# JessicaLeu-code/MotionPlanning_5D_m

Measured on AMD Instinct MI355X. Metric: CFS iterations/sec, 5-DoF 30-wp 8-obs batch-1024; l_inf wp err vs quadprog, higher is better.
Workload: dtype f64

## Files before the change

### motionplanning_5d_m_amd/csrc/cfs_device.h

```cpp
#pragma once
#include <hip/hip_runtime.h>
#include <stdint.h>
#include "../../include/cfs_hip.h"

#define CFS_WAVE 64

struct DevRobot {
    int kind;
    int nlink;
    double dh_d[CFS_MAX_LINKS];
    double dh_a[CFS_MAX_LINKS];
    double ca[CFS_MAX_LINKS];
    double sa[CFS_MAX_LINKS];
    double th_off[CFS_MAX_LINKS];
    double base[3];
    double cap[CFS_MAX_LINKS * 6];
    double t2l[CFS_MAX_LINKS * 3];
    double shift_bound;
    double prune_tol;
};
static_assert(sizeof(DevRobot) % 8 == 0, "DevRobot is copied to LDS as doubles");

struct DevCost {
    double Qp[36], Qv[36], Rs[36];
    double qc, ws, wt, pad;
};
static_assert(sizeof(DevCost) % 8 == 0, "DevCost is read as doubles");

struct DistArmParams {
    const DevRobot *rb;
    int N, nobs, nj;
    const double *theta;
    const double *obs;
    double *d;
    int *linkid;
    double *pos;
    double *grad;
};
void launch_dist_arm(const DistArmParams &p, hipStream_t s);
void launch_dist_arm_grad(const DistArmParams &p, hipStream_t s);

struct OrderParams {
    const DevRobot *rb;
    int B, H, nj, nobs;
    int obs_stride;
    int wp_stride;
    const double *x_init;
    const double *obs;
    const double *margin;
    int *key;
    int *order;
};
void launch_order(const OrderParams &p, hipStream_t s);

struct DenseConParams {
    int B, H, nj, nobs;
    double dt;
    const double *dist, *grad;
    const double *u;
    const double *xR1;
    const double *lim, *margin;
    double *Ainq;
    double *binq;
    const double *plim;
};
void launch_dense_con(const DenseConParams &p, hipStream_t s);

struct ClearParams {
    const DevRobot *rb;
    int B, H, nj, nobs, S;
    int move;
    double dt;
    const double *x_, *u, *xR1, *obs;
    double *dist_wp, *dist_path, *dist_lower, *t_path;
    int *link_path;
    int obs_stride, out_stride;
    double rho[CFS_MAX_LINKS * CFS_MAX_LINKS];
};
hipError_t launch_clearance(const ClearParams &p, hipStream_t s);
void cfs_clear_build_rho(const DevRobot &rb, int nj, double *rho);

enum { QP_OK = 0, QP_INFEASIBLE = 2, QP_NUMERIC = 3 };

struct GemvParams {
    int B, nn;
    const double *M;
    const double *X;
    double *Y;
    double scale;
};
void launch_batched_gemv(const GemvParams &p, hipStream_t s);

struct FusedParams {
    const DevRobot *rb;
    int B, H, nobs, mode, has_bounds, max_o_iter, noise_rows;
    int qy, lin_w;
    unsigned rc_nseg, rc_tile, rc_last;
    double dt, alpha, epsilon_O;
    double lmax_vel;
    double polish_tol;
    double lmax_H;
    const double *M1, *M2, *M3;
    const double *QQ;
    const DevCost *cost;
    const double *lim, *maxin, *margin;
    const double *x_init, *xR1, *ff, *caug, *obs, *noise;
    const double *x0;
    double *u, *x_, *cost_all, *e_cost_all, *e_u_all;
    int *iter_O, *total_iter, *status;
    double *Yg;
    double *Pt;
    size_t pt_stride;
    int *pool_flag;
    int pool_n;
    double *dbg;
    int dbg_b, dbg_cap;
    const int *order;
    unsigned long long *stamps;
    int opt;
    double *u_hist;
    double *u_log;
    int nmesh;
    const double *ext_dist;
    const double *ext_grad;
    int resume;
    int max_launch_iters;
    double *st_qu;
    double *st_cost;
    int *st_noise, *st_done;
    int warm_max;
    int piece;
    int no_prune;
    double *dump_dist;
    double *dump_grad;
    int *dump_linkid;
    double *dump_lambda;
};
struct SoftParams {
    double inv_weight;
    double *viol;
    int *n_soft;
};
enum FusedTier { FUSED_W1, FUSED_W2M, FUSED_W2S };
template <FusedTier T, bool JAC, bool SOFT, bool MOVE, bool LIM>
hipError_t launch_fused_tier(int nj, FusedParams p, hipStream_t s, const SoftParams *sp);
template <FusedTier T> bool fused_fits_tier(int nj, int H, int nobs, bool move = false, bool lim = false);
hipError_t launch_fused(int nj, FusedParams p, hipStream_t s, bool force_w1 = false, bool analytic = false, const SoftParams *soft = nullptr,
                        bool move = false, bool lim = false);
bool fused_fits(int nj, int H, int nobs);
bool fused_fits_move(int nj, int H, int nobs, int mode, bool lim = false);
bool fused_fits_lim(int nj, int H, int nobs, int mode, bool move);

struct CostHistParams {
    int B, nn, max_o_iter;
    const double *u_hist, *qu_hist;
    const double *ff, *caug;
    const int *iter_O;
    double *cost_all, *e_cost_all;
};
void launch_cost_history(const CostHistParams &p, hipStream_t s);

struct TermsParams {
    int B, H, nj;
    const double *F1, *F2;
    const double *Cq;
    const double *x0, *xg;
    const double *route;
    int nwp;
    const int *nwp_b;
    int nwp_stride;
    double dt;
    double *x_init, *xR1, *ff, *caug;
};
void launch_build_terms(const TermsParams &p, hipStream_t s);
```

### motionplanning_5d_m_amd/csrc/cfs_fused.hip

```cpp
#include "cfs_geom_dev.h"
#include <algorithm>
#include <atomic>
#include <type_traits>

namespace {

#define STAMP_IF(k) if (P.stamps) { const unsigned long long t_ = clock64(); if (tid == 0) s_acc[k] += t_ - t0_; t0_ = t_; }
#define STAMP(k) do { STAMP_IF(k) } while (0)

constexpr int CERT_AT = 6;
#ifndef CFS_WG_PER_CU
#define CFS_WG_PER_CU 1
#endif
#ifndef CFS_MOVE
#define CFS_MOVE 0
#endif
#ifndef CFS_LIM
#define CFS_LIM 0
#endif
constexpr double REF_A = 1e-4;
constexpr double REF_B = 1e-9;
constexpr int MV_BATCH = 16;
#ifndef CFS_TU
#define CFS_TU 8
#endif
#ifndef CFS_PR
#define CFS_PR 64
#endif
#ifndef CFS_P_LDS
#define CFS_P_LDS 0
#endif
#if CFS_P_LDS
constexpr int P_LDS_MAX_QB = 160;
#endif
static_assert(CFS_PR % 8 == 0 && CFS_PR >= 8, "register-resident P columns come in chunks of 8");
constexpr int FT = 256;
constexpr double DEP_TOL_F = 1e-8;
enum { CT_COL = 0, CT_VELP = 1, CT_VELM = 2, CT_BNDP = 3, CT_BNDM = 4, CT_POSP = 5, CT_POSM = 6 };
__device__ __forceinline__ int mk_code(int type, int i, int jc) { return (type << 16) | (i << 8) | jc; }
__host__ __device__ constexpr unsigned rcp31(unsigned d) { return (unsigned)(0x80000000ull / d) + 1u; }
__device__ __forceinline__ int rcp_div(int e, unsigned rc) { return (int)__umulhi((unsigned)e << 1, rc); }
#define CFS_RCP_DECODE (CFS_WG_PER_CU > 1)

template <int CTRL, int RM>
__device__ __forceinline__ double dpp_f64(double old, double src)
{
    const int rl = __builtin_amdgcn_update_dpp(__double2loint(old), __double2loint(src), CTRL, RM, 0xf, false);
    const int rh = __builtin_amdgcn_update_dpp(__double2hiint(old), __double2hiint(src), CTRL, RM, 0xf, false);
    return __hiloint2double(rh, rl);
}
__device__ __forceinline__ double readlane_f64(double v, int lane)
{
    return __hiloint2double(__builtin_amdgcn_readlane(__double2hiint(v), lane), __builtin_amdgcn_readlane(__double2loint(v), lane));
}
__device__ __forceinline__ double wave_min(double v)
{
    v = fmin(v, dpp_f64<0x111, 0xf>(v, v));
    v = fmin(v, dpp_f64<0x112, 0xf>(v, v));
    v = fmin(v, dpp_f64<0x114, 0xf>(v, v));
    v = fmin(v, dpp_f64<0x118, 0xf>(v, v));
    v = fmin(v, dpp_f64<0x142, 0xa>(v, v));
    v = fmin(v, dpp_f64<0x143, 0xc>(v, v));
    return readlane_f64(v, 63);
}
__device__ __forceinline__ double wave_add(double v)
{
    v += dpp_f64<0x111, 0xf>(0.0, v);
    v += dpp_f64<0x112, 0xf>(0.0, v);
    v += dpp_f64<0x114, 0xf>(0.0, v);
    v += dpp_f64<0x118, 0xf>(0.0, v);
    v += dpp_f64<0x142, 0xa>(0.0, v);
    v += dpp_f64<0x143, 0xc>(0.0, v);
    return readlane_f64(v, 63);
}

__device__ __forceinline__ void sync_rows(bool one_wave)
{
    if (one_wave) {
        __builtin_amdgcn_fence(__ATOMIC_RELEASE, "wavefront");
        __builtin_amdgcn_wave_barrier();
        __builtin_amdgcn_fence(__ATOMIC_ACQUIRE, "wavefront");
    } else __syncthreads();
}

__device__ __forceinline__ void block_argmin(double &v, int &id, double *red, int tid)
{
    const double m = wave_min(v);
    const unsigned long long hit = __ballot(v == m);
    const int src = hit ? (int)__builtin_ctzll(hit) : 0;
    const int mid = __builtin_amdgcn_readlane(id, src);
    const int wv = tid >> 6;
    if ((tid & 63) == 0) { red[wv] = m; reinterpret_cast<int *>(red + FT / 64)[wv] = mid; }
    __syncthreads();
    double bm = red[0];
    int bi = reinterpret_cast<int *>(red + FT / 64)[0];
#pragma unroll
    for (int w = 1; w < FT / 64; ++w) {
        const double om = red[w];
        const int oi = reinterpret_cast<int *>(red + FT / 64)[w];
        if (om < bm) { bm = om; bi = oi; }
    }
    v = bm; id = bi;
}
__device__ __forceinline__ double block_sum(double v, double *red, int tid)
{
    const double s = wave_add(v);
    if ((tid & 63) == 0) red[tid >> 6] = s;
    __syncthreads();
    double t = red[0];
#pragma unroll
    for (int w = 1; w < FT / 64; ++w) t += red[w];
    return t;
}

__device__ __forceinline__ void block_sum4(double &a, double &b, double &c, double &d, double *red, int tid)
{
    const double sa = wave_add(a), sb = wave_add(b), sc = wave_add(c), sd = wave_add(d);
    if ((tid & 63) == 0) { const int w = tid >> 6; red[w] = sa; red[4 + w] = sb; red[8 + w] = sc; red[12 + w] = sd; }
    __syncthreads();
    a = (red[0] + red[1]) + (red[2] + red[3]);
    b = (red[4] + red[5]) + (red[6] + red[7]);
    c = (red[8] + red[9]) + (red[10] + red[11]);
    d = (red[12] + red[13]) + (red[14] + red[15]);
}

__device__ __forceinline__ void block_sum3(double &a, double &b, double &c, double *red, int tid)
{
    const double sa = wave_add(a), sb = wave_add(b), sc = wave_add(c);
    if ((tid & 63) == 0) { const int w = tid >> 6; red[w] = sa; red[4 + w] = sb; red[8 + w] = sc; }
    __syncthreads();
    a = (red[0] + red[1]) + (red[2] + red[3]);
    b = (red[4] + red[5]) + (red[6] + red[7]);
    double t = red[8];
#pragma unroll
    for (int w = 1; w < FT / 64; ++w) t += red[8 + w];
    c = t;
}

__device__ __forceinline__ double wave_scan_incl(double v)
{
    v += dpp_f64<0x111, 0xf>(0.0, v);
    v += dpp_f64<0x112, 0xf>(0.0, v);
    v += dpp_f64<0x114, 0xf>(0.0, v);
    v += dpp_f64<0x118, 0xf>(0.0, v);
    v += dpp_f64<0x142, 0xa>(0.0, v);
    v += dpp_f64<0x143, 0xc>(0.0, v);
    return v;
}

__device__ __forceinline__ double half_scan_incl(double v)
{
    v += dpp_f64<0x111, 0xf>(0.0, v);
    v += dpp_f64<0x112, 0xf>(0.0, v);
    v += dpp_f64<0x114, 0xf>(0.0, v);
    v += dpp_f64<0x118, 0xf>(0.0, v);
    v += dpp_f64<0x142, 0xa>(0.0, v);
    return v;
}

template <int NJ>
__device__ __forceinline__ void roll_lds(double *buf, int H, double dt, int tid)
{
    const int HN = H * NJ;
    if (H <= 32) {
        const int lane = tid & 31;
        for (int c = tid >> 5; c < NJ; c += 2 * (FT / 64)) {
            const double x = lane < H ? buf[lane * NJ + c] : 0.0;
            const double sv = dt * half_scan_incl(x);
            const double sp = dt * half_scan_incl(sv) - (0.5 * dt) * sv;
            if (lane < H) { buf[HN + lane * NJ + c] = sv; buf[2 * HN + lane * NJ + c] = sp; }
        }
        return;
    }
    const int lane = tid & 63, wv = tid >> 6;
    for (int c = wv; c < NJ; c += FT / 64) {
        const double x = lane < H ? buf[lane * NJ + c] : 0.0;
        const double sv = dt * wave_scan_incl(x);
        const double sp = dt * wave_scan_incl(sv) - (0.5 * dt) * sv;
        if (lane < H) { buf[HN + lane * NJ + c] = sv; buf[2 * HN + lane * NJ + c] = sp; }
    }
}

template <int NJ, bool LIM = false>
__device__ __forceinline__ double ndot(int code, const double *buf, const double *g, int H)
{
    const int type = code >> 16, i = (code >> 8) & 0xff, jc = code & 0xff, HN = H * NJ;
    if constexpr (LIM) {
        if (type == CT_POSP) return -buf[2 * HN + i * NJ + jc];
        if (type == CT_POSM) return buf[2 * HN + i * NJ + jc];
    }
    switch (type) {
    case CT_COL: {
        double s = 0.0;
#pragma unroll
        for (int c = 0; c < NJ; ++c) s += g[(jc * H + i) * NJ + c] * buf[2 * HN + i * NJ + c];
        return s;
    }
    case CT_VELP: return -buf[HN + i * NJ + jc];
    case CT_VELM: return buf[HN + i * NJ + jc];
    case CT_BNDP: return -buf[i * NJ + jc];
    default: return buf[i * NJ + jc];
    }
}

template <int NJ, bool LIM = false>
__device__ __forceinline__ double slack_of(int code, const double *xs, const double *g, const double *rhs,
                                           const double *lim, const double *v0, const double *maxin, int H, double *bnd,
                                           double dt = 0.0, const double *plim = nullptr)
{
    const int type = code >> 16, i = (code >> 8) & 0xff, jc = code & 0xff, HN = H * NJ;
    if constexpr (LIM) {
        if (type == CT_POSP || type == CT_POSM) {
            const double pos = v0[NJ + jc] + ((double)(i + 1) * dt) * v0[jc];
            if (type == CT_POSP) { const double bb = plim[NJ + jc] - pos; *bnd = bb; return bb - xs[2 * HN + i * NJ + jc]; }
            const double bb = pos - plim[jc]; *bnd = bb; return bb + xs[2 * HN + i * NJ + jc];
        }
    }
    switch (type) {
    case CT_COL: {
        const double rh = rhs[jc * H + i];
        double s = rh;
#pragma unroll
        for (int c = 0; c < NJ; ++c) s += g[(jc * H + i) * NJ + c] * xs[2 * HN + i * NJ + c];
        *bnd = rh;
        return s;
    }
    case CT_VELP: { const double bb = lim[jc] - v0[jc]; *bnd = bb; return bb - xs[HN + i * NJ + jc]; }
    case CT_VELM: { const double bb = lim[jc] + v0[jc]; *bnd = bb; return bb + xs[HN + i * NJ + jc]; }
    case CT_BNDP: { const double bb = maxin[i * NJ + jc]; *bnd = bb; return bb - xs[i * NJ + jc]; }
    default: { const double bb = maxin[i * NJ + jc]; *bnd = bb; return bb + xs[i * NJ + jc]; }
    }
}


__device__ __forceinline__ double ramp_sum(int a, int m)
{
    const int M = m + 1;
    return 0.5 * (double)(M * (2 * a + 1) - m * M);
}
__device__ __forceinline__ double ramp_dot(int a, int b, int m)
{
    const int M = m + 1;
    return 0.25 * (double)(M * (2 * a + 1) * (2 * b + 1) - 2 * (a + b + 1) * m * M + 2 * (m * M * (2 * m + 1) / 3));
}
template <int NJ, bool LIM = false>
__device__ __forceinline__ double gram_ident(int ca, int cp, const double *g, int H, double dt)
{
    const int ta = ca >> 16, ia = (ca >> 8) & 0xff, ja = ca & 0xff;
    const int tp = cp >> 16, ip = (cp >> 8) & 0xff, jp = cp & 0xff;
    const int m = min(ia, ip);
    if constexpr (LIM) {
        const bool pa = ta >= CT_POSP, pp = tp >= CT_POSP;
        if (pa || pp) {
            const double sa = (ta == CT_POSP || ta == CT_VELP) ? -1.0 : 1.0, sp = (tp == CT_POSP || tp == CT_VELP) ? -1.0 : 1.0;
            if (ta == CT_COL) return (sp * g[(ja * H + ia) * NJ + jp]) * ((dt * dt) * (dt * dt) * ramp_dot(ia, ip, m));
            if (tp == CT_COL) return (sa * g[(jp * H + ip) * NJ + ja]) * ((dt * dt) * (dt * dt) * ramp_dot(ia, ip, m));
            if (ja != jp) return 0.0;
            if (pa && pp) return (sa * sp) * ((dt * dt) * (dt * dt) * ramp_dot(ia, ip, m));
            return (sa * sp) * ((dt * dt * dt) * ramp_sum(pa ? ia : ip, m));
        }
    }
    if (ta == CT_COL && tp == CT_COL) {
        double dot = 0.0;
#pragma unroll
        for (int c = 0; c < NJ; ++c) dot += g[(ja * H + ia) * NJ + c] * g[(jp * H + ip) * NJ + c];
        return dot * ((dt * dt) * (dt * dt) * ramp_dot(ia, ip, m));
    }
    if (ta == CT_COL) return g[(ja * H + ia) * NJ + jp] * ((tp == CT_VELP ? -1.0 : 1.0) * (dt * dt * dt) * ramp_sum(ia, m));
    if (tp == CT_COL) return g[(jp * H + ip) * NJ + ja] * ((ta == CT_VELP ? -1.0 : 1.0) * (dt * dt * dt) * ramp_sum(ip, m));
    if (ja != jp) return 0.0;
    return ((ta == tp) ? 1.0 : -1.0) * (dt * dt) * (double)(m + 1);
}

#if CFS_P_LDS
template <int PR, int QB, bool IN_LDS = false>
#else
template <int PR, int QB>
#endif
struct PRow {
    static constexpr int TU = CFS_TU;
    double v[PR];
    __device__ __forceinline__ void zero(double *ptail, int a, int q)
    {
#pragma unroll
        for (int b = 0; b < PR; ++b) v[b] = 0.0;
        for (int b = PR; b < q; ++b) ptail[(b - PR) * QB + a] = 0.0;
    }
    __device__ __forceinline__ double dot(const double *vec, const double *ptail, int a, int q) const
    {
        double s = 0.0;
#pragma unroll
        for (int b0 = 0; b0 < PR; b0 += 8)
            if (b0 < q) {
#pragma unroll
                for (int jj = 0; jj < 8; ++jj) s += v[b0 + jj] * vec[b0 + jj];
                __builtin_amdgcn_sched_barrier(0);
            }
        int b = PR;
        for (; b + TU <= q; b += TU) {
            double t[TU];
#pragma unroll
            for (int jj = 0; jj < TU; ++jj) t[jj] = ptail[(b + jj - PR) * QB + a];
#pragma unroll
            for (int jj = 0; jj < TU; ++jj) s += t[jj] * vec[b + jj];
        }
        for (; b < q; ++b) s += ptail[(b - PR) * QB + a] * vec[b];
        return s;
    }
    __device__ __forceinline__ void axpy(double alpha, const double *vec, double *ptail, int a, int q)
    {
#pragma unroll
        for (int b0 = 0; b0 < PR; b0 += 8)
            if (b0 < q) {
#pragma unroll
                for (int jj = 0; jj < 8; ++jj) v[b0 + jj] += alpha * vec[b0 + jj];
                __builtin_amdgcn_sched_barrier(0);
            }
        int b = PR;
        for (; b + TU <= q; b += TU) {
// ... 225 lines not shown
    return L;
}

template <int NJ, int QB, bool IDENT, bool JAC, bool MOVE, bool LIM, class... Soft>
__global__ __launch_bounds__(FT, CFS_WG_PER_CU) void cfs_solve_fused_kernel(FusedParams P, Soft... soft_params)
{
    constexpr bool SOFT = sizeof...(Soft) > 0;
    static_assert(!SOFT || (sizeof...(Soft) == 1 && (std::is_same_v<Soft, SoftParams> && ...)), "Soft is empty or SoftParams");
    const SoftParams S{soft_params...};
    constexpr int NS = 2 * NJ, NVT = nvt(NJ), NE = 2 * NJ + 1;
    extern __shared__ __attribute__((aligned(16))) double lds[];
    const int b = P.order ? P.order[blockIdx.x] : (int)blockIdx.x, tid = threadIdx.x;
    const int H = P.H, nobs = P.nobs, HN = H * NJ, nn = HN, NX = H * NS;
    const double dt = P.dt;
    constexpr int PR = QB < CFS_PR ? QB : CFS_PR;
    const FusedLayout L = fused_layout(NJ, H, nobs, QB, PR, LIM);
    DevRobot *rb = reinterpret_cast<DevRobot *>(lds + L.rb);
    double *s_ob = lds + L.ob, *s_x = lds + L.x, *s_u = lds + L.u, *s_qu = lds + L.qu, *s_g = lds + L.g;
    double *s_rhs = lds + L.rhs, *xs = lds + L.xs, *s_up = lds + L.up, *wb = lds + L.wb, *zb = lds + L.zb;
    double *s_d = lds + L.d, *s_r = lds + L.r, *s_rho = lds + L.rho, *s_lam = lds + L.lam, *s_prow = lds + L.prow;
    int *s_act = reinterpret_cast<int *>(lds + L.act);
    int *s_free = reinterpret_cast<int *>(lds + L.fre);
    int *s_prev = reinterpret_cast<int *>(lds + L.prev);
    unsigned char *s_flag = reinterpret_cast<unsigned char *>(lds + L.flag);
    unsigned short *s_slot = reinterpret_cast<unsigned short *>(lds + L.slot);
    int *s_code = reinterpret_cast<int *>(lds + L.code);
    double *red_base = lds + L.red;
    int red_sel = 0;
#define red (red_base + 24 * (red_sel ^= 1))
    double *s_lim = lds + L.small, *s_v0 = s_lim + NJ, *s_th0 = s_v0 + NJ, *s_margin = s_th0 + 2 * NJ;
    double *s_plim = s_margin + nobs;
    double *s_mx = lds + L.mx;
    double *s_racc = lds + L.racc;
    int pool_slot;
    {
        int *pubp = reinterpret_cast<int *>(red_base + 63);
        if (tid == 0) {
            int sidx = (int)(((blockIdx.x * 0x9E3779B1u) >> 8) % (unsigned)P.pool_n);
            int probes = 0;
            while (atomicCAS(&P.pool_flag[sidx * 16], 0, 1) != 0) {
                sidx = sidx + 1 == P.pool_n ? 0 : sidx + 1;
                __builtin_amdgcn_s_sleep(2);
                if (++probes > (1 << 22)) { sidx = -1; break; }
            }
            pubp[0] = sidx;
        }
        __syncthreads();
        pool_slot = pubp[0];
        if (pool_slot < 0) {
            if (tid == 0 && P.piece == 0) { P.status[b] = CFS_NUMERIC; P.iter_O[b] = 1; P.total_iter[b] = 0; }
            return;
        }
    }
    double *const s_pt = P.Pt + (size_t)pool_slot * P.pt_stride;
    double *s_Y = lds + L.y;
    const int QY = P.qy;
    double *const Yg = P.Yg + (size_t)pool_slot * nn * nn;
    auto drop_pool = [&]() {
        __syncthreads();
        if (tid == 0) { __threadfence(); atomicExch(&P.pool_flag[pool_slot * 16], 0); }
    };
    int ncon = nobs * H + (P.has_bounds ? 4 : 2) * HN;
    if constexpr (LIM) ncon = nobs * H + 6 * HN;
    const int maxit = 8 * nn + 200;
    if constexpr (LIM) {
        for (int e = tid; e < nobs * H; e += FT) { const int j = e / H; s_code[e] = mk_code(CT_COL, e - j * H, j); }
    } else
    for (int e = tid; e < ncon; e += FT) {
        int code;
        if (e < nobs * H) { const int j = e / H; code = mk_code(CT_COL, e - j * H, j); }
        else {
            const int f2 = e - nobs * H, ty = f2 / HN, k = f2 - ty * HN, i = k / NJ;
            code = mk_code(1 + ty, i, k - i * NJ);
        }
        s_code[e] = code;
    }

    {
        const double *src = reinterpret_cast<const double *>(P.rb);
        for (int e = tid; e < (int)(sizeof(DevRobot) / 8); e += FT) lds[L.rb + e] = src[e];
        if constexpr (!MOVE)
            for (int e = tid; e < nobs * 6; e += FT) s_ob[e] = P.obs[(size_t)b * nobs * 6 + e];
        for (int e = tid; e < NX; e += FT) s_x[e] = P.x_init[(size_t)b * NX + e];
        for (int e = tid; e < HN; e += FT) { s_u[e] = 0.0; s_qu[e] = 0.0; s_mx[e] = P.has_bounds ? P.maxin[e] : 0.0; }
        if (tid < NJ) {
            s_lim[tid] = P.lim[tid];
            s_v0[tid] = P.xR1[(size_t)b * NS + NJ + tid];
            s_th0[tid] = P.xR1[(size_t)b * NS + tid];
        }
        if (tid < nobs) s_margin[tid] = P.margin[tid];
        if constexpr (LIM)
            if (tid < 2 * NJ) s_plim[tid] = P.lim[NJ + tid];
        if (P.cost) {
            const double *csrc = reinterpret_cast<const double *>(P.cost);
            for (int e = tid; e < (int)(sizeof(DevCost) / 8); e += FT) lds[L.cost + e] = csrc[e];
        }
    }
    __syncthreads();
    if (P.has_bounds)
        for (int e = tid; e < HN; e += FT) {
            const int i = e / NJ, c = e - i * NJ;
            double acc = 0.0;
            for (int k = 0; k <= i; ++k) acc += ((double)(i - k) + 0.5) * s_mx[k * NJ + c];
            s_racc[e] = (dt * dt) * acc;
        }
    unsigned long long *s_acc = reinterpret_cast<unsigned long long *>(red_base + 48);
    if (tid < 12) s_acc[tid] = 0ull;
    unsigned long long t0_ = P.stamps ? clock64() : 0ull;
    double cost_new = P.caug[b], cost_old = 100000.0;
    int iter_O = 1, total_iter = 0, noise_row = 0, status = CFS_OK_MAXITER;
    bool done = false;
    const double iw = S.inv_weight;
    int n_soft = 0;
    bool last_soft = false;
    const int nseg = nobs - P.nmesh;
    int launched = 0;
    if (P.resume) {
        for (int e = tid; e < NX; e += FT) s_x[e] = P.x_[(size_t)b * NX + e];
        for (int e = tid; e < HN; e += FT) { s_u[e] = P.u[(size_t)b * nn + e]; s_qu[e] = P.st_qu[(size_t)b * nn + e]; }
        cost_new = P.st_cost[2 * b]; cost_old = P.st_cost[2 * b + 1];
        iter_O = P.iter_O[b]; total_iter = P.total_iter[b]; status = P.status[b];
        noise_row = P.st_noise[b]; done = P.st_done[b] != 0;
        __syncthreads();
    } else if (P.piece == 0) {
        double d2 = 0.0;
        for (int e = tid; e < NX; e += FT) { const double v = s_x[e] - 1.0; d2 += v * v; }
        d2 = block_sum(d2, red, tid);
        if (sqrt(d2) < P.epsilon_O) { done = true; status = CFS_OK_CONVERGED; }
        else if (iter_O > P.max_o_iter) { done = true; status = CFS_OK_MAXITER; }
    } else if (P.piece == 2) {
        for (int e = tid; e < HN; e += FT) s_u[e] = P.u[(size_t)b * nn + e];
        __syncthreads();
    }

#if CFS_P_LDS
    PRow<PR, QB, QB <= P_LDS_MAX_QB> Pr;
#else
    PRow<PR, QB> Pr;
#endif
#if CFS_P_LDS
    static_assert(IDENT, "the P block takes the place of the Y rows: identity Hessian only");
    if constexpr (QB <= P_LDS_MAX_QB) Pr.pl = lds + L.pl;
#endif
    int prev_q = 0;

    while (!done) {
        bool skip = false;
        if (P.piece == 0 && P.mode == CFS_MODE_PSGCFS) {
            skip = fabs(cost_new - cost_old) < 1e-4;
            if (!skip) cost_old = cost_new;
        } else if (P.piece == 0) cost_old = cost_new;
        const int noise_row_now = noise_row;
        if (P.piece == 0 && P.mode == CFS_MODE_PSGCFS && !skip) ++noise_row;
        auto prep = [&](int ph) {
            if (P.piece == 1) return;
            if (ph == 0) { for (int k = tid; k < HN; k += FT) xs[k] = s_u[k]; }
            else if (ph == 1) roll_lds<NJ>(xs, H, dt, tid);
            else if (ph == 2) {
                const bool psg = P.piece == 0 && P.mode == CFS_MODE_PSGCFS;
                const double sc = (double)iter_O * (double)iter_O + 1.0;
                const bool have = P.noise != nullptr && noise_row_now < P.noise_rows;
                for (int k = tid; k < HN; k += FT) {
                    s_up[k] = xs[2 * HN + k];
                    double v;
                    if (psg && skip) v = s_u[k];
                    else if (psg) {
                        const double nz = have ? P.noise[((size_t)b * P.noise_rows + noise_row_now) * nn + k] : 0.0;
                        v = s_u[k] - P.alpha * ((s_qu[k] + P.ff[(size_t)b * nn + k]) + 10.0 * nz / sc);
                    } else v = P.x0[(size_t)b * nn + k];
                    xs[k] = v;
                }
            } else roll_lds<NJ>(xs, H, dt, tid);
        };
        bool prepped = false;
        if constexpr (JAC) {
            if (nseg > 0) {
                const int W = P.lin_w;
                double *s_sc = lds + L.lin;
                double *s_en = s_sc + W * NJ * 6;
                double *s_tw = s_en + W * NJ * 6;
                double *s_bd = s_en + W * NVT * 6;
#define S_OBW (s_bd + W * NJ * nseg)
                for (int w0 = 0; w0 < H; w0 += W) {
                    const int Wc = min(W, H - w0);
#if CFS_RCP_DECODE
                    unsigned rc_n = P.rc_nseg, rc_t = Wc == W ? P.rc_tile : P.rc_last;
                    asm volatile("" : "+s"(rc_n), "+s"(rc_t));
#endif
                    if (w0 == 0) prep(0);
                    if constexpr (MOVE)
                        for (int e = tid; e < Wc * nseg * 6; e += FT) S_OBW[e] = P.obs[((size_t)b * H + w0) * nobs * 6 + e];
                    for (int e = tid; e < Wc * NJ; e += FT) {
                        const int m = e % NJ, wi = e / NJ;
                        double x = s_x[(w0 + wi) * NS + m];
                        x = x - rb->th_off[m];
                        double sn, cs;
                        sincos(x, &sn, &cs);
                        s_sc[e * 2] = sn;
                        s_sc[e * 2 + 1] = cs;
                    }
                    __syncthreads();
                    for (int wi = tid; wi < Wc; wi += FT) arm_chain(rb, NJ, s_sc + wi * NJ * 2, s_en + wi * NJ * 6, s_tw + wi * NJ * 6);
                    if (w0 == 0) prep(1);
                    __syncthreads();
                    STAMP(10);
                    for (int e = tid; e < NJ * Wc * nseg; e += FT) {
#if CFS_RCP_DECODE
                        const int q = rcp_div(e, rc_n), j = e - q * nseg, k0 = rcp_div(e, rc_t), wi = q - k0 * Wc;
#else
                        const int j = e % nseg, wi = (e / nseg) % Wc, k0 = e / (nseg * Wc);
#endif
                        if constexpr (MOVE) s_bd[(wi * NJ + k0) * nseg + j] = seg_seg_dist(s_en + (wi * NJ + k0) * 6, S_OBW + (wi * nseg + j) * 6);
                        else s_bd[(wi * NJ + k0) * nseg + j] = seg_seg_dist(s_en + (wi * NJ + k0) * 6, s_ob + j * 6);
                    }
                    if (w0 == 0) prep(2);
                    __syncthreads();
                    STAMP(0);
                    for (int e = tid; e < Wc * nseg; e += FT) {
#if CFS_RCP_DECODE
                        const int wi = rcp_div(e, rc_n), j = e - wi * nseg;
#else
                        const int j = e % nseg, wi = e / nseg;
#endif
                        double m0 = INFINITY;
                        int lk = 0;
#pragma unroll
                        for (int k1 = 1; k1 <= NJ; ++k1) { const double bk = s_bd[(wi * NJ + k1 - 1) * nseg + j]; if (bk < m0) { m0 = bk; lk = k1; } }
                        if (P.dump_linkid && launched == 0) P.dump_linkid[((size_t)b * nobs + j) * H + w0 + wi] = lk;
                        s_rhs[j * H + w0 + wi] = m0;
                        double *g = s_g + (j * H + w0 + wi) * NJ;
                        if constexpr (MOVE) {
                            if (lk > 0) winner_grad(s_en + (wi * NJ + lk - 1) * 6, s_tw + wi * NJ * 6, lk - 1, NJ, S_OBW + (wi * nseg + j) * 6, g);
                            else for (int m = 0; m < NJ; ++m) g[m] = 0.0;
                        } else {
                            if (lk > 0) winner_grad(s_en + (wi * NJ + lk - 1) * 6, s_tw + wi * NJ * 6, lk - 1, NJ, s_ob + j * 6, g);
                            else for (int m = 0; m < NJ; ++m) g[m] = 0.0;
                        }
                    }
                    if (w0 == 0) { prep(3); prepped = true; }
                    if constexpr (MOVE) __syncthreads();
                    else if (w0 + W >= H) __syncthreads();
                    STAMP(11);
                }
#undef S_OBW
            }
        } else {
            if (nseg > 0) {
                const int W = P.lin_w;
                double *s_sc = lds + L.lin;
                double *s_en = s_sc + W * NJ * 6;
                double *s_bd = s_en + W * NVT * 6;
                double *s_dv = s_bd + W * NJ * nseg;
                unsigned short *s_list = reinterpret_cast<unsigned short *>(s_dv + W * nseg * NE);
#define S_OBW (s_dv + W * nseg * NE + (NJ * W * nseg + 3) / 4)
                int *s_cnt = s_free;
                for (int w0 = 0; w0 < H; w0 += W) {
                    const int Wc = min(W, H - w0);
#if CFS_RCP_DECODE
                    unsigned rc_n = P.rc_nseg, rc_t = Wc == W ? P.rc_tile : P.rc_last;
                    asm volatile("" : "+s"(rc_n), "+s"(rc_t));
#endif
                    if (w0 == 0) prep(0);
                    if constexpr (MOVE)
                        for (int e = tid; e < Wc * nseg * 6; e += FT) S_OBW[e] = P.obs[((size_t)b * H + w0) * nobs * 6 + e];
                    for (int e = tid; e < Wc * NJ * 3; e += FT) {
                        const int var = e % 3, m = (e / 3) % NJ, wi = e / (3 * NJ);
                        double x = s_x[(w0 + wi) * NS + m];
                        if (var == 1) x = x + FD_EPS / 2;
                        else if (var == 2) x = x - FD_EPS / 2;
                        x = x - rb->th_off[m];
                        double sn, cs;
                        sincos(x, &sn, &cs);
                        s_sc[((wi * NJ + m) * 3 + var) * 2] = sn;
                        s_sc[((wi * NJ + m) * 3 + var) * 2 + 1] = cs;
                    }
                    __syncthreads();
                    for (int e = tid; e < Wc * NE; e += FT) {
                        const int ev = e % NE, wi = e / NE;
                        double M[12], Mn[12], e6[6];
#pragma unroll
                        for (int k1 = 1; k1 <= NJ; ++k1) {
                            const int avar = (ev == 2 * k1 - 1) ? 1 : (ev >= 2 * k1 ? 2 : 0);
                            const double sn = s_sc[((wi * NJ + k1 - 1) * 3 + avar) * 2], cs = s_sc[((wi * NJ + k1 - 1) * 3 + avar) * 2 + 1];
                            fk_step(rb, k1 - 1, sn, cs, k1 == 1 ? nullptr : M, Mn);
#pragma unroll
                            for (int qq = 0; qq < 12; ++qq) M[qq] = Mn[qq];
                            if (ev <= 2 * k1) {
                                link_ends(rb, k1 - 1, M, e6);
                                double *dstE = s_en + (wi * NVT + kvoff(k1) + ev) * 6;
#pragma unroll
                                for (int qq = 0; qq < 6; ++qq) dstE[qq] = e6[qq];
                            }
                        }
                    }
                    if (w0 == 0) prep(1);
                    __syncthreads();
                    STAMP(10);
                    for (int e = tid; e < NJ * Wc * nseg; e += FT) {
#if CFS_RCP_DECODE
                        const int q = rcp_div(e, rc_n), j = e - q * nseg, k0 = rcp_div(e, rc_t), wi = q - k0 * Wc;
#else
                        const int j = e % nseg, wi = (e / nseg) % Wc, k0 = e / (nseg * Wc);
#endif
                        if constexpr (MOVE) s_bd[(wi * NJ + k0) * nseg + j] = seg_seg_dist(s_en + (wi * NVT + kvoff(k0 + 1)) * 6, S_OBW + (wi * nseg + j) * 6);
                        else s_bd[(wi * NJ + k0) * nseg + j] = seg_seg_dist(s_en + (wi * NVT + kvoff(k0 + 1)) * 6, s_ob + j * 6);
                    }
                    if (tid < NJ) s_cnt[tid] = 0;
                    if (w0 == 0) prep(2);
                    __syncthreads();
                    for (int e = tid; e < Wc * nseg; e += FT) {
#if CFS_RCP_DECODE
                        const int wi = rcp_div(e, rc_n), j = e - wi * nseg;
#else
                        const int j = e % nseg, wi = e / nseg;
#endif
                        double bk[NJ], m0 = INFINITY;
                        int lk = 0;
#pragma unroll
                        for (int k1 = 1; k1 <= NJ; ++k1) { bk[k1 - 1] = s_bd[(wi * NJ + k1 - 1) * nseg + j]; if (bk[k1 - 1] < m0) { m0 = bk[k1 - 1]; lk = k1; } }
                        if (P.dump_linkid && launched == 0) P.dump_linkid[((size_t)b * nobs + j) * H + w0 + wi] = lk;
                        const double thr = P.no_prune ? INFINITY : fmax(m0, 0.0001) + rb->prune_tol;
#pragma unroll
                        for (int k1 = 1; k1 <= NJ; ++k1)
                            if (bk[k1 - 1] < thr) s_list[(k1 - 1) * W * nseg + atomicAdd(&s_cnt[k1 - 1], 1)] = (unsigned short)((wi << 8) | j);
                        s_dv[e * NE] = m0;
#pragma unroll
                        for (int ev = 1; ev < NE; ++ev) s_dv[e * NE + ev] = INFINITY;
                    }
                    if (w0 == 0) { prep(3); prepped = true; }
                    __syncthreads();
                    STAMP(0);
                    {
                        int offs[NJ + 1];
                        offs[0] = 0;
#pragma unroll
                        for (int k1 = 1; k1 <= NJ; ++k1) offs[k1] = offs[k1 - 1] + s_cnt[k1 - 1] * 2 * k1;
                        for (int e = tid; e < offs[NJ]; e += FT) {
#if CFS_RCP_DECODE
                            int k1 = 1, lo = 0;
                            unsigned rc = 0x80000001u;
#pragma unroll
                            for (int kk = 2; kk <= NJ; ++kk)
                                if (e >= offs[kk - 1]) { k1 = kk; lo = offs[kk - 1]; rc = (unsigned)(0x100000000ull / (2 * kk)) + 1u; }
                            const int r_ = e - lo, ent = (int)__umulhi((unsigned)r_, rc), v = r_ - ent * (2 * k1) + 1;
#else
                            int k1 = 1, ent = 0, v = 1;
#pragma unroll
                            for (int kk = 1; kk <= NJ; ++kk)
                                if (e >= offs[kk - 1] && e < offs[kk]) {
                                    const int r_ = e - offs[kk - 1];
                                    k1 = kk; ent = r_ / (2 * kk); v = r_ - ent * (2 * kk) + 1;
                                }
#endif
                            const int item = s_list[(k1 - 1) * W * nseg + ent], wi = item >> 8, j = item & 255;
                            double dis;
                            if constexpr (MOVE) dis = seg_seg_dist(s_en + (wi * NVT + kvoff(k1) + v) * 6, S_OBW + (wi * nseg + j) * 6);
                            else dis = seg_seg_dist(s_en + (wi * NVT + kvoff(k1) + v) * 6, s_ob + j * 6);
                            double *dv = s_dv + (wi * nseg + j) * NE;
                            const int evhi = (v == 2 * k1) ? NE - 1 : v;
                            for (int ev = v; ev <= evhi; ++ev)
                                __hip_atomic_fetch_min(dv + ev, dis, __ATOMIC_RELAXED, __HIP_MEMORY_SCOPE_WORKGROUP);
                        }
                    }
                    __syncthreads();
                    STAMP(11);
                    for (int e = tid; e < Wc * nseg; e += FT) {
#if CFS_RCP_DECODE
                        const int wi = rcp_div(e, rc_n), j = e - wi * nseg;
#else
                        const int j = e % nseg, wi = e / nseg;
#endif
                        double dev[NE];
#pragma unroll
                        for (int ev = 0; ev < NE; ++ev) dev[ev] = s_dv[e * NE + ev];
                        s_rhs[j * H + w0 + wi] = dev[0];
#pragma unroll
                        for (int m = 0; m < NJ; ++m) s_g[(j * H + w0 + wi) * NJ + m] = (dev[2 * m + 1] - dev[2 * m + 2]) / FD_EPS;
                    }
                    if (w0 + W >= H) __syncthreads();
                }
#undef S_OBW
            }
        }
        if (!prepped && P.piece != 1) {
            prep(0); __syncthreads(); prep(1); __syncthreads(); prep(2); __syncthreads(); prep(3); __syncthreads();
        }

        if (P.nmesh > 0) {
            for (int e = tid; e < P.nmesh * H; e += FT) s_rhs[nseg * H + e] = P.ext_dist[(size_t)b * P.nmesh * H + e];
            for (int e = tid; e < P.nmesh * HN; e += FT) s_g[nseg * HN + e] = P.ext_grad[(size_t)b * P.nmesh * HN + e];
            __syncthreads();
        }

        if (P.dump_dist && launched == 0) {
            for (int e = tid; e < nobs * H; e += FT) P.dump_dist[(size_t)b * nobs * H + e] = s_rhs[e];
            for (int e = tid; e < nobs * HN; e += FT) P.dump_grad[(size_t)b * nobs * HN + e] = s_g[e];
        }
        if (P.piece == 1) { drop_pool(); return; }

        STAMP(0);
        int qp_status = QP_OK, iters = 0;
        int qhi = 0, nfree = 0;
        int npolish = 0;
        auto n_combine = [&](const double *coef, const double *base, int pc_) {
            const int ptype_ = pc_ >> 16, pi_ = (pc_ >> 8) & 0xff, pj_ = pc_ & 0xff;
            const bool two = H <= 32;
            const int lane = two ? (tid & 31) : (tid & 63);
            const int iR = H - 1 - lane;
            const int cstep = two ? 2 * (FT / 64) : FT / 64;
            for (int c = two ? (tid >> 5) : (tid >> 6); c < NJ; c += cstep) {
                double Rp = 0.0, Rv = 0.0;
                if (lane < H) {
                    const int sp_ = s_slot[nobs * H + iR * NJ + c], sm_ = s_slot[nobs * H + HN + iR * NJ + c];
                    for (int j0 = 0; j0 < nobs; j0 += 8) {
                        int sl[8];
#pragma unroll
                        for (int jj = 0; jj < 8; ++jj) sl[jj] = j0 + jj < nobs ? s_slot[(j0 + jj) * H + iR] : 0;
#pragma unroll
                        for (int jj = 0; jj < 8; ++jj)
                            if (sl[jj]) Rp += coef[sl[jj] - 1] * s_g[((j0 + jj) * H + iR) * NJ + c];
                    }
                    if (sp_) Rv -= dt * coef[sp_ - 1];
                    if (sm_) Rv += dt * coef[sm_ - 1];
                    if constexpr (LIM) {
                        const int pp_ = s_slot[nobs * H + 4 * HN + iR * NJ + c], pm_ = s_slot[nobs * H + 5 * HN + iR * NJ + c];
                        if (pp_) Rp -= coef[pp_ - 1];
                        if (pm_) Rp += coef[pm_ - 1];
                    }
                }
                const double S1 = two ? half_scan_incl(Rp) : wave_scan_incl(Rp);
                const double cmb = (dt * dt) * S1 + Rv;
                const double S2V = two ? half_scan_incl(cmb) : wave_scan_incl(cmb);
                const double nr_rev = S2V - (0.5 * dt * dt) * S1;
                const int src = (lane < H ? H - 1 - lane : lane) + (two ? (tid & 32) : 0);
                const double nr = __shfl(nr_rev, src, 64);
                double z0 = 0.0;
                if (lane < H) {
                    if (base) z0 = base[lane * NJ + c];
                    else if (ptype_ == CT_COL) z0 = lane <= pi_ ? s_g[(pj_ * H + pi_) * NJ + c] * ((dt * dt) * ((double)(pi_ - lane) + 0.5)) : 0.0;
                    else z0 = (c == pj_ && lane <= pi_) ? (ptype_ == CT_VELP ? -dt : dt) : 0.0;
                    if constexpr (LIM)
                        if (!base && ptype_ >= CT_POSP)
                            z0 = (c == pj_ && lane <= pi_) ? (ptype_ == CT_POSP ? -1.0 : 1.0) * ((dt * dt) * ((double)(pi_ - lane) + 0.5)) : 0.0;
                    z0 -= nr;
                }
                const double sv = dt * (two ? half_scan_incl(z0) : wave_scan_incl(z0));
                const double spo = dt * (two ? half_scan_incl(sv) : wave_scan_incl(sv)) - (0.5 * dt) * sv;
                if (lane < H) { zb[lane * NJ + c] = z0; zb[HN + lane * NJ + c] = sv; zb[2 * HN + lane * NJ + c] = spo; }
            }
        };
        auto y_combine = [&](const double *coef, const double *base) {
            const int qa = min(qhi, QY);
            for (int k = tid; k < HN; k += FT) {
                double z0 = base ? base[k] : 0.0, z1 = 0.0, z2 = 0.0, z3 = 0.0;
                int a = 0;
                for (; a + 4 <= qa; a += 4) {
                    z0 -= coef[a] * s_Y[a * HN + k];
                    z1 -= coef[a + 1] * s_Y[(a + 1) * HN + k];
                    z2 -= coef[a + 2] * s_Y[(a + 2) * HN + k];
                    z3 -= coef[a + 3] * s_Y[(a + 3) * HN + k];
                }
                for (; a < qa; ++a) z0 -= coef[a] * s_Y[a * HN + k];
                for (a = qa; a + CFS_TU <= qhi; a += CFS_TU) {
                    double t[CFS_TU];
#pragma unroll
                    for (int jj = 0; jj < CFS_TU; ++jj) t[jj] = Yg[(size_t)(a + jj) * nn + k];
#pragma unroll
                    for (int jj = 0; jj < CFS_TU; jj += 4) {
                        z0 -= coef[a + jj] * t[jj]; z1 -= coef[a + jj + 1] * t[jj + 1]; z2 -= coef[a + jj + 2] * t[jj + 2]; z3 -= coef[a + jj + 3] * t[jj + 3];
                    }
                }
                for (; a < qhi; ++a) z0 -= coef[a] * Yg[(size_t)a * nn + k];
                zb[k] = (z0 + z1) + (z2 + z3);
            }
        };
        auto y_combine_roll = [&](const double *coef, const double *base) {
            const int lane = tid & 31;
            for (int c = tid >> 5; c < NJ; c += 2 * (FT / 64)) {
                const int k = lane * NJ + c;
                double z0 = 0.0, z1 = 0.0, z2 = 0.0, z3 = 0.0;
                if (lane < H) {
                    z0 = base ? base[k] : 0.0;
// ... 574 lines not shown
                    const double y_rev = S2V - (0.5 * dt * dt) * S1;
                    const int src = (lane < H ? H - 1 - lane : lane) + (two ? (tid & 32) : 0);
                    const double y = __shfl(y_rev, src, 64);
                    if (lane < H) {
                        const int k = lane * NJ + c;
                        double ru = 0.0;
#pragma unroll
                        for (int c2 = 0; c2 < NJ; ++c2) ru += ck->Rs[c + c2 * NJ] * xs[lane * NJ + c2];
                        const double sq = y + ru;
                        s_qu[k] = sq;
                        cpart += xs[k] * (0.5 * sq + P.ff[(size_t)b * nn + k]);
                    }
                }
            } else
            for (int k = tid; k < HN; k += FT) {
                double sa[8] = {0.0, 0.0, 0.0, 0.0, 0.0, 0.0, 0.0, 0.0};
                int c = 0;
                for (; c + MV_BATCH <= HN; c += MV_BATCH) {
                    double ld[MV_BATCH];
#pragma unroll
                    for (int j = 0; j < MV_BATCH; ++j) ld[j] = P.QQ[k + (size_t)(c + j) * nn];
#pragma unroll
                    for (int j = 0; j < MV_BATCH; ++j) sa[j & 7] += ld[j] * xs[c + j];
                }
                for (; c < HN; ++c) sa[0] += P.QQ[k + (size_t)c * nn] * xs[c];
                const double s = ((sa[0] + sa[1]) + (sa[2] + sa[3])) + ((sa[4] + sa[5]) + (sa[6] + sa[7]));
                s_qu[k] = s;
                cpart += xs[k] * (0.5 * s + P.ff[(size_t)b * nn + k]);
            }
        }
        block_sum3(du2, dx2, cpart, red, tid);
        if (P.u_hist) {
            if (tid == 0) P.e_u_all[(size_t)b * P.max_o_iter + (iter_O - 1)] = sqrt(du2);
        } else {
            cost = cpart + P.caug[b];
            if (tid == 0) {
                const size_t o = (size_t)b * P.max_o_iter + (iter_O - 1);
                P.cost_all[o] = cost;
                P.e_cost_all[o] = fabs(cost_old - cost);
                P.e_u_all[o] = sqrt(du2);
            }
        }
        STAMP(9);
        cost_new = cost;
        ++iter_O;
        if (sqrt(dx2) < P.epsilon_O) { done = true; status = CFS_OK_CONVERGED; }
        else if (iter_O > P.max_o_iter) { done = true; status = CFS_OK_MAXITER; }
        if (P.max_launch_iters > 0 && ++launched >= P.max_launch_iters) break;
    }

    drop_pool();
    __syncthreads();
    for (int e = tid; e < HN; e += FT) P.u[(size_t)b * nn + e] = s_u[e];
    for (int e = tid; e < NX; e += FT) P.x_[(size_t)b * NX + e] = s_x[e];
    if constexpr (SOFT) {
        if (last_soft && (status == CFS_OK_CONVERGED || status == CFS_OK_MAXITER)) status = CFS_SOFT_ENDED;
        if (tid == 0 && S.n_soft) S.n_soft[b] = n_soft;
    }
    if (tid == 0) { P.iter_O[b] = iter_O; P.total_iter[b] = total_iter; P.status[b] = status; }
    if (P.st_qu) {
        for (int e = tid; e < HN; e += FT) P.st_qu[(size_t)b * nn + e] = s_qu[e];
        if (tid == 0) { P.st_cost[2 * b] = cost_new; P.st_cost[2 * b + 1] = cost_old; P.st_noise[b] = noise_row; P.st_done[b] = done ? 1 : 0; }
    }
    if (P.stamps && tid == 0) for (int k = 0; k < 12; ++k) P.stamps[(size_t)b * 12 + k] = s_acc[k];
}

#undef red

template <int NJ, int QB, bool IDENT, bool JAC, bool SOFT, bool MOVE, bool LIM>
hipError_t launch_fused_inst2(const FusedParams &p, size_t lds, hipStream_t s, const SoftParams *sp)
{
    static std::atomic<unsigned long long> attr_set{0ull};
    using Kernel = std::conditional_t<SOFT, void (*)(FusedParams, SoftParams), void (*)(FusedParams)>;
    const Kernel kern = cfs_solve_fused_kernel<NJ, QB, IDENT, JAC, MOVE, LIM>;
    int dev = 0;
    hipError_t e = hipGetDevice(&dev);
    if (e != hipSuccess) return e;
    if (dev >= 64 || !((attr_set.load(std::memory_order_acquire) >> dev) & 1ull)) {
        e = hipFuncSetAttribute(reinterpret_cast<const void *>(kern), hipFuncAttributeMaxDynamicSharedMemorySize, 160 * 1024);
        if (e != hipSuccess) return e;
        if (dev < 64) attr_set.fetch_or(1ull << dev, std::memory_order_release);
    }
    if constexpr (SOFT) hipLaunchKernelGGL(kern, dim3(p.B), dim3(FT), lds, s, p, *sp);
    else hipLaunchKernelGGL(kern, dim3(p.B), dim3(FT), lds, s, p);
    return hipGetLastError();
}

#ifndef CFS_IDENT_SET
#define CFS_IDENT_SET 2
#endif
template <int NJ, int QB, bool JAC, bool SOFT, bool MOVE, bool LIM>
hipError_t launch_fused_inst(const FusedParams &p, size_t lds, hipStream_t s, const SoftParams *sp)
{
    const bool ident = p.mode == CFS_MODE_PSGCFS;
#if CFS_IDENT_SET != 0
    if (ident) return launch_fused_inst2<NJ, QB, true, JAC, SOFT, MOVE, LIM>(p, lds, s, sp);
#endif
#if CFS_IDENT_SET != 1
    if (!ident) return launch_fused_inst2<NJ, QB, false, JAC, SOFT, MOVE, LIM>(p, lds, s, sp);
#endif
    return hipErrorInvalidValue;
}

struct FusedPlan {
    int nn, QB;
    FusedLayout L;
    size_t avail, per_wp;
};
FusedPlan fused_plan(int nj, int H, int nobs, bool move, bool lim = false)
{
    FusedPlan q;
    q.nn = H * nj;
    q.QB = q.nn <= 96 ? 96 : (q.nn <= 160 ? 160 : 256);
    q.L = fused_layout(nj, H, nobs, q.QB, q.QB < CFS_PR ? q.QB : CFS_PR, lim);
    q.avail = (160 * 1024 / CFS_WG_PER_CU) / 8 - 64;
    q.per_wp = (size_t)nj * 6 + (size_t)nvt(nj) * 6 + (size_t)nj * nobs + (size_t)nobs * (2 * nj + 1) + ((size_t)nj * nobs + 3) / 4;
    if (move) q.per_wp += (size_t)nobs * 6;
    return q;
}

}

template <FusedTier T>
bool fused_fits_tier(int nj, int H, int nobs, bool move, bool lim)
{
    const FusedPlan q = fused_plan(nj, H, nobs, move, lim);
    return (size_t)q.L.total_fixed + (size_t)4 * q.nn <= q.avail && (size_t)q.L.lin + q.per_wp <= q.avail;
}

template <FusedTier T, bool JAC, bool SOFT, bool MOVE, bool LIM>
hipError_t launch_fused_tier(int nj, FusedParams p, hipStream_t s, const SoftParams *sp)
{
    if (MOVE && p.nmesh > 0) return hipErrorInvalidValue;
    const FusedPlan q = fused_plan(nj, p.H, p.nobs, MOVE);
    const int nn = q.nn;
    const FusedLayout &L = q.L;
    const bool ident = p.mode == CFS_MODE_PSGCFS;
    if ((size_t)L.total_fixed + (ident ? 0 : 4 * nn) > q.avail) return hipErrorInvalidValue;
    const size_t region = q.avail - L.total_fixed;
    int qy = ident ? 0 : (int)(region / nn);
    if (qy > nn) qy = nn;
    int w = (int)((q.avail - L.lin) / q.per_wp);
    if (w < 1) return hipErrorInvalidValue;
    w = (p.H + (p.H + w - 1) / w - 1) / ((p.H + w - 1) / w);
    p.qy = qy;
    p.lin_w = w;
    {
        const int nseg = p.nobs - p.nmesh, wl = p.H - (p.H - 1) / w * w;
        p.rc_nseg = p.rc_tile = p.rc_last = 0;
        if (nseg > 0) {
            if ((unsigned long long)nj * w * nseg * ((unsigned long long)w * nseg) >= 0x80000000ull) return hipErrorInvalidValue;
            p.rc_nseg = rcp31(nseg); p.rc_tile = rcp31(nseg * w); p.rc_last = rcp31(nseg * wl);
        }
    }
    size_t need = std::max((size_t)L.total_fixed + (size_t)qy * nn, (size_t)L.lin + (size_t)w * q.per_wp);
    if constexpr (LIM) {
        const FusedPlan ql = fused_plan(nj, p.H, p.nobs, MOVE, true);
        need = std::max((size_t)ql.L.total_fixed + (size_t)qy * nn, (size_t)ql.L.lin + (size_t)w * ql.per_wp);
        if (need > ql.avail) return hipErrorInvalidValue;
    }
    const size_t lds = need * 8;
    switch (nj * 1000 + q.QB) {
    case 2096: return launch_fused_inst<2, 96, JAC, SOFT, MOVE, LIM>(p, lds, s, sp);
    case 3096: return launch_fused_inst<3, 96, JAC, SOFT, MOVE, LIM>(p, lds, s, sp);
    case 4096: return launch_fused_inst<4, 96, JAC, SOFT, MOVE, LIM>(p, lds, s, sp);
    case 5096: return launch_fused_inst<5, 96, JAC, SOFT, MOVE, LIM>(p, lds, s, sp);
    case 6096: return launch_fused_inst<6, 96, JAC, SOFT, MOVE, LIM>(p, lds, s, sp);
    case 2160: return launch_fused_inst<2, 160, JAC, SOFT, MOVE, LIM>(p, lds, s, sp);
    case 4160: return launch_fused_inst<4, 160, JAC, SOFT, MOVE, LIM>(p, lds, s, sp);
    case 5160: return launch_fused_inst<5, 160, JAC, SOFT, MOVE, LIM>(p, lds, s, sp);
    case 6160: return launch_fused_inst<6, 160, JAC, SOFT, MOVE, LIM>(p, lds, s, sp);
    case 3160: return launch_fused_inst<3, 160, JAC, SOFT, MOVE, LIM>(p, lds, s, sp);
    case 3256: return launch_fused_inst<3, 256, JAC, SOFT, MOVE, LIM>(p, lds, s, sp);
    case 4256: return launch_fused_inst<4, 256, JAC, SOFT, MOVE, LIM>(p, lds, s, sp);
    case 5256: return launch_fused_inst<5, 256, JAC, SOFT, MOVE, LIM>(p, lds, s, sp);
    case 6256: return launch_fused_inst<6, 256, JAC, SOFT, MOVE, LIM>(p, lds, s, sp);
    default: return hipErrorInvalidValue;
    }
}

template hipError_t launch_fused_tier<CFS_TIER, CFS_JAC, CFS_SOFT, CFS_MOVE, CFS_LIM>(int, FusedParams, hipStream_t, const SoftParams *);
#if !CFS_JAC && !CFS_SOFT && !CFS_MOVE && !CFS_LIM
template bool fused_fits_tier<CFS_TIER>(int, int, int, bool, bool);
#endif
```

Measured before the change: 11.04 million.

## Run prep phases on waves left idle by ragged geometry loops

The host computes, for each geometry phase, how many leading waves finish a round early given the loop trip count, and packs these counts into a new ride field. The prep work (roll scan, noise/state update) interleaved with those phases is then shifted onto the trailing waves by offsetting its start index and stride. The aim is to hide prep latency inside the tail of the ragged geometry loops rather than stacking it on top. It only compiles in when multiple workgroups per CU and LDS-resident P are both enabled, so it may be inactive under default build flags.

```diff
diff --git a/motionplanning_5d_m_amd/csrc/cfs_device.h b/motionplanning_5d_m_amd/csrc/cfs_device.h
--- a/motionplanning_5d_m_amd/csrc/cfs_device.h
+++ b/motionplanning_5d_m_amd/csrc/cfs_device.h
@@ -96,6 +96,7 @@
     int B, H, nobs, mode, has_bounds, max_o_iter, noise_rows;
     int qy, lin_w;
     unsigned rc_nseg, rc_tile, rc_last;
+    unsigned ride;
     double dt, alpha, epsilon_O;
     double lmax_vel;
     double polish_tol;
diff --git a/motionplanning_5d_m_amd/csrc/cfs_fused.hip b/motionplanning_5d_m_amd/csrc/cfs_fused.hip
--- a/motionplanning_5d_m_amd/csrc/cfs_fused.hip
+++ b/motionplanning_5d_m_amd/csrc/cfs_fused.hip
@@ -41,6 +41,7 @@
 __host__ __device__ constexpr unsigned rcp31(unsigned d) { return (unsigned)(0x80000000ull / d) + 1u; }
 __device__ __forceinline__ int rcp_div(int e, unsigned rc) { return (int)__umulhi((unsigned)e << 1, rc); }
 #define CFS_RCP_DECODE (CFS_WG_PER_CU > 1)
+#define CFS_RIDE_IDLE (CFS_WG_PER_CU > 1 && CFS_P_LDS)
 
 template <int CTRL, int RM>
 __device__ __forceinline__ double dpp_f64(double old, double src)
@@ -159,12 +160,13 @@
 }
 
 template <int NJ>
-__device__ __forceinline__ void roll_lds(double *buf, int H, double dt, int tid)
+__device__ __forceinline__ void roll_lds(double *buf, int H, double dt, int tid, int first = 0)
 {
     const int HN = H * NJ;
     if (H <= 32) {
         const int lane = tid & 31;
-        for (int c = tid >> 5; c < NJ; c += 2 * (FT / 64)) {
+        const int c0 = (tid >> 5) - 2 * first;
+        for (int c = c0 < 0 ? NJ : c0; c < NJ; c += 2 * (FT / 64 - first)) {
             const double x = lane < H ? buf[lane * NJ + c] : 0.0;
             const double sv = dt * half_scan_incl(x);
             const double sp = dt * half_scan_incl(sv) - (0.5 * dt) * sv;
@@ -696,15 +698,24 @@
         } else if (P.piece == 0) cost_old = cost_new;
         const int noise_row_now = noise_row;
         if (P.piece == 0 && P.mode == CFS_MODE_PSGCFS && !skip) ++noise_row;
-        auto prep = [&](int ph) {
+        auto prep = [&](int ph, bool riding = false) {
             if (P.piece == 1) return;
+            int first = 0;
+#if CFS_RIDE_IDLE
+            if (riding) {
+                unsigned rd = P.ride;
+                asm volatile("" : "+s"(rd));
+                first = (int)((rd >> (4 * ph)) & 15u);
+            }
+#endif
             if (ph == 0) { for (int k = tid; k < HN; k += FT) xs[k] = s_u[k]; }
-            else if (ph == 1) roll_lds<NJ>(xs, H, dt, tid);
+            else if (ph == 1) roll_lds<NJ>(xs, H, dt, tid, first);
             else if (ph == 2) {
                 const bool psg = P.piece == 0 && P.mode == CFS_MODE_PSGCFS;
                 const double sc = (double)iter_O * (double)iter_O + 1.0;
                 const bool have = P.noise != nullptr && noise_row_now < P.noise_rows;
-                for (int k = tid; k < HN; k += FT) {
+                const int k0 = tid - 64 * first;
+                for (int k = k0 < 0 ? HN : k0; k < HN; k += FT - 64 * first) {
                     s_up[k] = xs[2 * HN + k];
                     double v;
                     if (psg && skip) v = s_u[k];
@@ -714,7 +725,7 @@
                     } else v = P.x0[(size_t)b * nn + k];
                     xs[k] = v;
                 }
-            } else roll_lds<NJ>(xs, H, dt, tid);
+            } else roll_lds<NJ>(xs, H, dt, tid, first);
         };
         bool prepped = false;
         if constexpr (JAC) {
@@ -745,7 +756,7 @@
                     }
                     __syncthreads();
                     for (int wi = tid; wi < Wc; wi += FT) arm_chain(rb, NJ, s_sc + wi * NJ * 2, s_en + wi * NJ * 6, s_tw + wi * NJ * 6);
-                    if (w0 == 0) prep(1);
+                    if (w0 == 0) prep(1, true);
                     __syncthreads();
                     STAMP(10);
                     for (int e = tid; e < NJ * Wc * nseg; e += FT) {
@@ -757,7 +768,7 @@
                         if constexpr (MOVE) s_bd[(wi * NJ + k0) * nseg + j] = seg_seg_dist(s_en + (wi * NJ + k0) * 6, S_OBW + (wi * nseg + j) * 6);
                         else s_bd[(wi * NJ + k0) * nseg + j] = seg_seg_dist(s_en + (wi * NJ + k0) * 6, s_ob + j * 6);
                     }
-                    if (w0 == 0) prep(2);
+                    if (w0 == 0) prep(2, true);
                     __syncthreads();
                     STAMP(0);
                     for (int e = tid; e < Wc * nseg; e += FT) {
@@ -781,7 +792,7 @@
                             else for (int m = 0; m < NJ; ++m) g[m] = 0.0;
                         }
                     }
-                    if (w0 == 0) { prep(3); prepped = true; }
+                    if (w0 == 0) { prep(3, true); prepped = true; }
                     if constexpr (MOVE) __syncthreads();
                     else if (w0 + W >= H) __syncthreads();
                     STAMP(11);
@@ -837,7 +848,7 @@
                             }
                         }
                     }
-                    if (w0 == 0) prep(1);
+                    if (w0 == 0) prep(1, true);
                     __syncthreads();
                     STAMP(10);
                     for (int e = tid; e < NJ * Wc * nseg; e += FT) {
@@ -850,7 +861,7 @@
                         else s_bd[(wi * NJ + k0) * nseg + j] = seg_seg_dist(s_en + (wi * NVT + kvoff(k0 + 1)) * 6, s_ob + j * 6);
                     }
                     if (tid < NJ) s_cnt[tid] = 0;
-                    if (w0 == 0) prep(2);
+                    if (w0 == 0) prep(2, true);
                     __syncthreads();
                     for (int e = tid; e < Wc * nseg; e += FT) {
 #if CFS_RCP_DECODE
@@ -871,7 +882,7 @@
 #pragma unroll
                         for (int ev = 1; ev < NE; ++ev) s_dv[e * NE + ev] = INFINITY;
                     }
-                    if (w0 == 0) { prep(3); prepped = true; }
+                    if (w0 == 0) { prep(3, true); prepped = true; }
                     __syncthreads();
                     STAMP(0);
                     {
@@ -1752,6 +1763,15 @@
             if ((unsigned long long)nj * w * nseg * ((unsigned long long)w * nseg) >= 0x80000000ull) return hipErrorInvalidValue;
             p.rc_nseg = rcp31(nseg); p.rc_tile = rcp31(nseg * w); p.rc_last = rcp31(nseg * wl);
         }
+        auto first_free = [](int n) {
+            const int p0 = (n + FT - 1) / FT;
+            for (int v = 1; v < FT / 64; ++v)
+                if ((n > 64 * v ? (n - 64 * v + FT - 1) / FT : 0) < p0) return (unsigned)v;
+            return 0u;
+        };
+        p.ride = 0;
+        if (nseg > 0 && p.H <= 32)
+            p.ride = first_free(JAC ? w : w * (2 * nj + 1)) << 4 | first_free(nj * w * nseg) << 8 | first_free(w * nseg) << 12;
     }
     size_t need = std::max((size_t)L.total_fixed + (size_t)qy * nn, (size_t)L.lin + (size_t)w * q.per_wp);
     if constexpr (LIM) {
```

Measured after the change: 11.16 million (median of 6 runs). 1.1% higher.
